# pymc-devs/nuts-rs

Measured on AMD Instinct MI355X. Metric: leapfrog-steps*dims/sec at 4096 chains x dim 1024 (post-warm-up NUTS draws), higher is better.
Workload: dtype f64; 1 GPU; K2: iid N(3,1) dim 1024 x 4096 chains per GPU, maxdepth 10, per-chain diag mass matrix, DiagNutsSettings defaults, num_tune 400 (untimed), seed 20260928; chains_per_gpu=4096, dim=1024, num_tune=400, parallelism=chains sharded x1, no collective, rng=ChaCha8 stream + ziggurat normals (reference semantics), draws_recorded=True, recorded_buffers_verified=True

## Files before the change

nuts_rs_amd/csrc/dev_math.hpp:

```cpp
#pragma once
#include <hip/hip_runtime.h>
#include <stdint.h>
#include "nuts_contract.hpp"
#include "detmath_tables.hpp"

namespace nm {

#define NM_DEV __device__ __forceinline__

#define NM_HD __host__ __device__ __forceinline__
NM_HD uint64_t d2u(double x) { return __builtin_bit_cast(uint64_t, x); }
NM_HD double u2d(uint64_t u) { return __builtin_bit_cast(double, u); }
#ifndef NM_TILE_MODE
#define NM_TILE_MODE 0
#endif
#define NM_ONE_WAVE_BLOCK (NM_TILE_MODE || blockDim.x == 64)
NM_DEV int lane_id() { return (int)(threadIdx.x & 63); }
NM_DEV void block_sync(bool single_wave) {
    if (single_wave || NM_TILE_MODE) asm volatile("" ::: "memory");
    else __syncthreads();
}
NM_DEV void chain_sync() { block_sync(false); }
NM_DEV int tid() { return NM_TILE_MODE ? (int)(threadIdx.x & 63) : (int)threadIdx.x; }
NM_DEV int wave_id() { return __builtin_amdgcn_readfirstlane((int)(threadIdx.x >> 6)); }
// ... 712 lines not shown
NM_DEV double fmin_rs(double a, double b) { return __builtin_fmin(a, b); }

NM_DEV void chacha8_block(const uint32_t* key, uint64_t counter, uint64_t stream, uint32_t (&out)[16]) {
    uint32_t s[16] = {0x61707865u, 0x3320646eu, 0x79622d32u, 0x6b206574u,
                      key[0], key[1], key[2], key[3], key[4], key[5], key[6], key[7],
                      (uint32_t)counter, (uint32_t)(counter >> 32), (uint32_t)stream, (uint32_t)(stream >> 32)};
    uint32_t x[16];
#pragma unroll
    for (int i = 0; i < 16; ++i) x[i] = s[i];
#define NM_QR(a, b, c, d)                                                   \
    x[a] += x[b]; x[d] ^= x[a]; x[d] = __builtin_rotateleft32(x[d], 16);    \
    x[c] += x[d]; x[b] ^= x[c]; x[b] = __builtin_rotateleft32(x[b], 12);    \
    x[a] += x[b]; x[d] ^= x[a]; x[d] = __builtin_rotateleft32(x[d], 8);     \
    x[c] += x[d]; x[b] ^= x[c]; x[b] = __builtin_rotateleft32(x[b], 7);
#pragma unroll
    for (int r = 0; r < 4; ++r) {
        NM_QR(0, 4, 8, 12) NM_QR(1, 5, 9, 13) NM_QR(2, 6, 10, 14) NM_QR(3, 7, 11, 15)
        NM_QR(0, 5, 10, 15) NM_QR(1, 6, 11, 12) NM_QR(2, 7, 8, 13) NM_QR(3, 4, 9, 14)
    }
#undef NM_QR
#pragma unroll
    for (int i = 0; i < 16; ++i) out[i] = x[i] + s[i];
}

constexpr int RNG_CACHE_WORDS = 512;
struct DevRng {
    const uint32_t* key;
    uint64_t pos;
    uint64_t base;
    uint32_t* cache;
    uint32_t cap;
    bool one_wave;

    NM_DEV void init(const uint32_t* k, uint64_t p, uint32_t* lds) {
        one_wave = NM_ONE_WAVE_BLOCK;
        key = k;
        pos = p;
        base = p + 16;
        cache = lds;
        cap = RNG_CACHE_WORDS;
    }
    NM_DEV bool has(uint64_t nwords) const { return pos >= base && (pos - base) + nwords <= (uint64_t)cap; }
    NM_DEV void refill() {
        block_sync(one_wave);
        base = pos & ~15ull;
        cap = RNG_CACHE_WORDS;
        if (tid() < RNG_CACHE_WORDS / 16) {
            uint32_t out[16];
            chacha8_block(key, (base >> 4) + (uint64_t)tid(), 0ull, out);
            uint4* dst = reinterpret_cast<uint4*>(cache + tid() * 16);
            dst[0] = make_uint4(out[0], out[1], out[2], out[3]);
            dst[1] = make_uint4(out[4], out[5], out[6], out[7]);
            dst[2] = make_uint4(out[8], out[9], out[10], out[11]);
            dst[3] = make_uint4(out[12], out[13], out[14], out[15]);
        }
        block_sync(one_wave);
    }
    NM_DEV uint32_t next_u32() {
        if (!has(1)) refill();
        uint32_t w = cache[pos - base];
        pos += 1;
        return w;
    }
    NM_DEV uint64_t next_u64() {
        if (!has(2)) refill();
        uint64_t lo = cache[pos - base], hi = cache[pos - base + 1];
        pos += 2;
        return (hi << 32) | lo;
    }
    NM_DEV bool random_bool_std() { return (int32_t)next_u32() < 0; }
    NM_DEV double random_f64() { return (double)(next_u64() >> 11) * (1.0 / 9007199254740992.0); }
    NM_DEV int random_bool(double p) {
        if (!(p >= 0.0 && p < 1.0)) return p == 1.0 ? 1 : -1;
        uint64_t p_int = (uint64_t)(p * 18446744073709551616.0);
        return next_u64() < p_int ? 1 : 0;
    }
};

struct ZigTables { const double* x; const double* f; };
constexpr double ZIG_R = 3.654152885361008796;

NM_DEV double normal_slow_path(DevRng& rng, uint64_t bits, ZigTables T) {
    for (;;) {
        int i = (int)(bits & 0xff);
        double u = u2d((bits >> 12) | 0x4000000000000000ull) - 3.0;
        double x = u * T.x[i];
        if (__builtin_fabs(x) < T.x[i + 1]) return x;
        if (i == 0) {
            double xx = 1.0, yy = 0.0;
            while (-2.0 * yy < xx * xx) {
                double a = u2d((rng.next_u64() >> 12) | 0x3ff0000000000000ull) - (1.0 - 2.220446049250313e-16 / 2.0);
                double b = u2d((rng.next_u64() >> 12) | 0x3ff0000000000000ull) - (1.0 - 2.220446049250313e-16 / 2.0);
                xx = ulog(a) / ZIG_R;
                yy = ulog(b);
            }
            return u < 0.0 ? xx - ZIG_R : ZIG_R - xx;
        }
        if (T.f[i + 1] + (T.f[i] - T.f[i + 1]) * rng.random_f64() < uexp(-x * x / 2.0)) return x;
        bits = rng.next_u64();
    }
}

NM_DEV void fill_standard_normals(DevRng& rng, double* stage, int count, ZigTables T) {
    const int lane = lane_id();
    int i = 0;
    while (i < count) {
        if (!rng.has(128)) rng.refill();
        const int nvalid = (count - i) < 64 ? (count - i) : 64;
        const uint32_t off = (uint32_t)(rng.pos - rng.base) + 2u * (uint32_t)lane;
        uint64_t bits = ((uint64_t)rng.cache[off + 1] << 32) | rng.cache[off];
        int zi = (int)(bits & 0xff);
        double u = u2d((bits >> 12) | 0x4000000000000000ull) - 3.0;
        double x = u * T.x[zi];
        bool ok = __builtin_fabs(x) < T.x[zi + 1];
        uint64_t fail = __ballot(lane < nvalid && !ok);
        int nacc = fail ? (int)__builtin_ctzll(fail) : nvalid;
        if (lane < nacc) stage[i + lane] = x;
        rng.pos += 2ull * (uint64_t)nacc;
        i += nacc;
        if (fail) {
            uint64_t fbits = wave_bcast_u64(bits, nacc);
            rng.pos += 2;
            double xs = normal_slow_path(rng, fbits, T);
            if (lane == 0) stage[i] = xs;
            i += 1;
        }
    }
    chain_sync();
}

constexpr int ZIG_FMAX = 64;
NM_DEV int uniform_i32(int x) { return __builtin_amdgcn_readfirstlane(x); }
NM_DEV int lane_get(int v, int idx) { return __builtin_amdgcn_readlane(v, idx); }
NM_DEV double lane_get_f64(double v, int idx) {
    const uint64_t b = d2u(v);
    const uint32_t lo = (uint32_t)__builtin_amdgcn_readlane((int)(uint32_t)b, idx);
    const uint32_t hi = (uint32_t)__builtin_amdgcn_readlane((int)(uint32_t)(b >> 32), idx);
    return u2d(((uint64_t)hi << 32) | lo);
}

#ifndef NM_PROF
#define NM_PROF 0
#endif
#if NM_PROF
#define NM_MARK_F(slot)                                                           \
    {                                                                             \
        const unsigned long long now_ = __builtin_amdgcn_s_memtime();             \
        if (blockIdx.x == 0 && threadIdx.x == 0) (void)__hip_atomic_fetch_add(&prof[slot], now_ - prof_t, __ATOMIC_RELAXED, __HIP_MEMORY_SCOPE_AGENT);     \
        prof_t = now_;                                                            \
    }
#else
#define NM_MARK_F(slot)
#endif
template <int P>
NM_DEV void fill_standard_normals_bulk(DevRng& rng, uint32_t* wbuf, double* samp, int count, ZigTables T, int nthreads,
                                       unsigned long long* prof, unsigned long long& prof_t) {
    static_assert(P <= 64, "rejection masks are kept one per lane");
    const int lane = lane_id();
    uint32_t* const small_cache = rng.cache;
    int produced = 0;
    block_sync(nthreads == 64);
    while (produced < count) {
        const int need = count - produced;
        int nc = need + ((need >> 4) > 8 ? (need >> 4) : 8);
        if (nc > 64 * P) nc = 64 * P;
        const uint64_t pos0 = rng.pos;
        const uint64_t b0 = pos0 >> 4;
        const int nb = (int)(((pos0 + 2ull * (uint64_t)nc - 1ull) >> 4) - b0) + 1;
        uint64_t* const lmask = reinterpret_cast<uint64_t*>(small_cache + 256);
        if (lane < 2 * P) lmask[lane] = 0ull;
        for (int b = tid(); b < nb; b += nthreads) {
            uint32_t out[16];
            chacha8_block(rng.key, b0 + (uint64_t)b, 0ull, out);
            uint4* dst = reinterpret_cast<uint4*>(wbuf + b * 16);
            dst[0] = make_uint4(out[0], out[1], out[2], out[3]);
            dst[1] = make_uint4(out[4], out[5], out[6], out[7]);
            dst[2] = make_uint4(out[8], out[9], out[10], out[11]);
            dst[3] = make_uint4(out[12], out[13], out[14], out[15]);
        }
        block_sync(nthreads == 64);
        NM_MARK_F(8)
        rng.cache = wbuf; rng.base = b0 << 4; rng.cap = (uint32_t)nb * 16u;
        const int w0 = (int)(pos0 - rng.base);
        double xr[P];
        int* const flist = reinterpret_cast<int*>(small_cache);
        int nrej = 0;
        {
            uint64_t cb[P];
            double tx[P], tn[P];
#pragma unroll
            for (int p = 0; p < P; ++p) {
                const int c = 64 * p + lane;
                cb[p] = ((uint64_t)wbuf[w0 + 2 * c + 1] << 32) | wbuf[w0 + 2 * c];
            }
#pragma unroll
            for (int p = 0; p < P; ++p) {
                const int zi = (int)(cb[p] & 0xff);
                tx[p] = T.x[zi];
                tn[p] = T.x[zi + 1];
            }
#pragma unroll
            for (int p = 0; p < P; ++p) {
                const int c = 64 * p + lane;
                const double u = u2d((cb[p] >> 12) | 0x4000000000000000ull) - 3.0;
                const double x = u * tx[p];
                const bool rej = !(__builtin_fabs(x) < tn[p]) && c < nc;
                xr[p] = x;
                const uint64_t fail = __ballot(rej);
                const int rank = nrej + (int)__builtin_amdgcn_mbcnt_hi((uint32_t)(fail >> 32),
                                                                       __builtin_amdgcn_mbcnt_lo((uint32_t)fail, 0u));
                flist[(rej && rank < ZIG_FMAX) ? rank : ZIG_FMAX + lane] = c;
                nrej += (int)__builtin_popcountll(fail);
            }
        }
        const int nlist = nrej < ZIG_FMAX ? nrej : ZIG_FMAX;
        int fcell, sp_r;
        double sp_x;
        bool sp_scalar;
        fcell = 0; sp_r = 0; sp_x = 0.0; sp_scalar = false;
        if (nlist > 0) {
            fcell = lane < nlist ? flist[lane] : 0;
            const int wa = w0 + 2 * fcell;
            const uint64_t bits0 = ((uint64_t)wbuf[wa + 1] << 32) | wbuf[wa];
            const uint64_t bits1 = ((uint64_t)wbuf[wa + 3] << 32) | wbuf[wa + 2];
            const uint64_t bits2 = ((uint64_t)wbuf[wa + 5] << 32) | wbuf[wa + 4];
            const int i0 = (int)(bits0 & 0xff);
            const double u0 = u2d((bits0 >> 12) | 0x4000000000000000ull) - 3.0;
            const double x0 = u0 * T.x[i0];
            const double u01 = (double)(bits1 >> 11) * (1.0 / 9007199254740992.0);
            const bool wedge = T.f[i0 + 1] + (T.f[i0] - T.f[i0 + 1]) * u01 < dexp(-x0 * x0 / 2.0);
            const int i2 = (int)(bits2 & 0xff);
            const double u2 = u2d((bits2 >> 12) | 0x4000000000000000ull) - 3.0;
            const double x2 = u2 * T.x[i2];
            const bool ok2 = __builtin_fabs(x2) < T.x[i2 + 1];
            sp_r = wedge ? 1 : 2;
            sp_x = wedge ? x0 : x2;
            sp_scalar = i0 == 0 || fcell + 2 >= nc || (!wedge && !ok2);
        }
        NM_MARK_F(9)
        NM_MARK_F(12)
        int cur = 0, j = 0, nf = 0;
        uint64_t sw = 0, nk = 0;
        int flj = 0;
        double flx = 0.0;
        bool open = true;
        const uint64_t scalar_mask = __ballot(sp_scalar);
        const int rr = lane < nlist ? sp_r : 0;
        const uint64_t m1 = __ballot(rr == 1), m2 = __ballot(rr == 2);
        const int s_before = (int)__builtin_amdgcn_mbcnt_hi((uint32_t)(m1 >> 32), __builtin_amdgcn_mbcnt_lo((uint32_t)m1, 0u)) +
                             2 * (int)__builtin_amdgcn_mbcnt_hi((uint32_t)(m2 >> 32), __builtin_amdgcn_mbcnt_lo((uint32_t)m2, 0u));
        const int prev_end = __builtin_amdgcn_update_dpp(-1, fcell + rr, 0x138, 0xf, 0xf, false);
        const bool chained = lane >= 1 && lane < nlist && fcell <= prev_end;
        const bool fast = scalar_mask == 0ull && nrej <= nlist && __ballot(chained) == 0ull;
        bool ev_active = false;
        int ev_j = 0;
        if (fast) {
            ev_j = fcell - s_before;
            ev_active = lane < nlist && ev_j < need;
            const uint64_t am = __ballot(ev_active);
            const int s_act = (int)__builtin_popcountll(m1 & am) + 2 * (int)__builtin_popcountll(m2 & am);
            j = (nc - s_act) < need ? (nc - s_act) : need;
            cur = j + s_act;
            if (ev_active) {
                const int q = fcell >> 6, off = fcell & 63;
                const uint64_t nk0 = ((1ull << (rr + 1)) - 1ull) << off;
                const uint64_t sw0 = off == 63 ? 0ull : (((1ull << rr) - 1ull) << (off + 1));
                (void)__hip_atomic_fetch_or(&lmask[q], sw0, __ATOMIC_RELAXED, __HIP_MEMORY_SCOPE_WORKGROUP);
                (void)__hip_atomic_fetch_or(&lmask[P + q], nk0, __ATOMIC_RELAXED, __HIP_MEMORY_SCOPE_WORKGROUP);
                const int spill = off + rr + 1 - 64;
                if (spill > 0) {
                    const uint64_t nx = (1ull << spill) - 1ull;
                    (void)__hip_atomic_fetch_or(&lmask[q + 1], nx, __ATOMIC_RELAXED, __HIP_MEMORY_SCOPE_WORKGROUP);
                    (void)__hip_atomic_fetch_or(&lmask[P + q + 1], nx, __ATOMIC_RELAXED, __HIP_MEMORY_SCOPE_WORKGROUP);
                }
            }
            sw = lane < P ? lmask[lane] : 0ull;
            nk = lane < P ? lmask[P + lane] : 0ull;
            open = false;
        }
        for (int g = 0; g < nlist && !fast; ++g) {
            const int f = lane_get(fcell, g);
            if (f < cur) continue;
            if (j + (f - cur) >= need) { cur += need - j; j = need; open = false; break; }
            j += f - cur;
            int r;
            double xs;
            if ((scalar_mask >> g) & 1ull) {
                const uint32_t lo = (uint32_t)uniform_i32((int)wbuf[w0 + 2 * f]);
                const uint32_t hi = (uint32_t)uniform_i32((int)wbuf[w0 + 2 * f + 1]);
                rng.pos = pos0 + 2ull * (uint64_t)(f + 1);
                xs = normal_slow_path(rng, ((uint64_t)hi << 32) | lo, T);
                r = (int)((rng.pos - pos0) >> 1) - (f + 1);
            } else {
                r = lane_get(sp_r, g);
                xs = lane_get_f64(sp_x, g);
            }
            for (int a = f, end = (f + 1 + r < 64 * P ? f + 1 + r : 64 * P); a < end;) {
                const int q = a >> 6, off = a & 63;
                const int take = (end - a) < (64 - off) ? (end - a) : (64 - off);
                const uint64_t bits = (take >= 64 ? ~0ull : ((1ull << take) - 1ull)) << off;
                const uint64_t sbits = a == f ? (bits & ~(1ull << off)) : bits;
                nk |= lane == q ? bits : 0ull;
                sw |= lane == q ? sbits : 0ull;
                a += take;
            }
            flj = lane == nf ? j : flj;
            flx = lane == nf ? xs : flx;
            nf += 1;
            j += 1;
            cur = f + 1 + r;
            if (j >= need || cur >= nc) { open = false; break; }
        }
        if (nrej > nlist && !fast) open = false;
        if (open && cur < nc) {
            const int take = (nc - cur) < (need - j) ? (nc - cur) : (need - j);
            j += take; cur += take;
        }
        rng.pos = pos0 + 2ull * (uint64_t)cur;
        NM_MARK_F(10)
        {
            double* const dummy = reinterpret_cast<double*>(small_cache) + 64 + lane;
            const int swlo = (int)(uint32_t)sw, swhi = (int)(uint32_t)(sw >> 32);
            const int nklo = (int)(uint32_t)nk, nkhi = (int)(uint32_t)(nk >> 32);
            int base = 0;
#pragma unroll
            for (int p = 0; p < P; ++p) {
                const uint32_t s_lo = (uint32_t)lane_get(swlo, p), s_hi = (uint32_t)lane_get(swhi, p);
                const uint64_t n_p = ((uint64_t)(uint32_t)lane_get(nkhi, p) << 32) | (uint32_t)lane_get(nklo, p);
                const int c = 64 * p + lane;
                const int below = (int)__builtin_amdgcn_mbcnt_hi(s_hi, __builtin_amdgcn_mbcnt_lo(s_lo, 0u));
                const bool keep = !((n_p >> lane) & 1ull) && c < cur;
                double* dst = keep ? samp + (produced + c - base - below) : dummy;
                *dst = xr[p];
                base += (int)__builtin_popcount(s_lo) + (int)__builtin_popcount(s_hi);
            }
            double* dst = fast ? (ev_active ? samp + (produced + ev_j) : dummy) : (lane < nf ? samp + (produced + flj) : dummy);
            *dst = fast ? sp_x : flx;
        }
        produced += j;
        block_sync(nthreads == 64);
// ... 24 lines not shown
```

nuts_rs_amd/csrc/nuts_kernels.hpp:

```cpp
#pragma once
#include <type_traits>
#include "nuts_contract.hpp"
#include "dev_math.hpp"
#include "../../include/nuts_amd.h"

namespace nm {

#ifndef NM_LDS_L1
#define NM_LDS_L1 1
#endif
constexpr int NM_CHECK_GROUP = 2;
#define NM_GROUP_BARRIER(m) do { if (((m) + 1) % NM_CHECK_GROUP == 0) __builtin_amdgcn_sched_barrier(0); } while (0)

constexpr bool plain_unit = !NM_TILE_MODE && !NM_CLUSTER_MODE;
template <int DPL, int W> constexpr bool reg_edges() { return plain_unit && W == 1 && (DPL == 16 || DPL == 2); }
template <int DPL, int W> constexpr bool batched_merges() { return batched_merges(DPL, W, plain_unit); }
template <int DPL, int W, class Dens> constexpr bool nog_mode();
constexpr int NM_TEST_CHUNK = 4;
constexpr int NM_TEST_CHUNK3_MAX = 2;

#ifndef NM_PROF
#define NM_PROF 0
#endif
#if NM_PROF
// ... 837 lines not shown
                o.v.a[k] = vh;
                o.z.a[k] = __builtin_fma(epsilon, vh, s.z.a[k]);
            }
            transform_to_x(C, o.z, x);
            o.logp = C.dens.template eval<DPL, W>(x, gx, C.dim, C.red);
            transform_to_gz(C, gx, o.g);
            double acc = 0.0;
#pragma unroll
            for (int k = 0; k < DPL; ++k) {
                o.v.a[k] = __builtin_fma(half, o.g.a[k], o.v.a[k]);
                acc = __builtin_fma(o.v.a[k], o.v.a[k], acc);
            }
            o.ke = 0.5 * C.red.sum(acc);
            if (x_out) *x_out = x;
            if (gx_out) *gx_out = gx;
            return;
        }
    }
    const double2* sg2 = C.tptr(C.lsig);
    const double2* mu2 = C.tptr(C.lmu);
    if constexpr (elementwise_trait<Dens>::value && plain_unit) {
        double acc = 0.0, kacc = 0.0;
        auto pass = [&](auto full_tile) __attribute__((always_inline)) {
            constexpr bool FULL = decltype(full_tile)::value;
            double2 sg = sg2[0], mm = mu2[0];
            [[maybe_unused]] double2 gg = make_double2(0., 0.);
            if constexpr (GMODE == 2) gg = C.ld2(gsrc.r, gsrc.so, 0);
#pragma unroll
            for (int m = 0; m < DPL / 2; ++m) {
                const double2 sg_c = sg, mm_c = mm;
                [[maybe_unused]] const double2 gg_c = gg;
                if (m + 1 < DPL / 2) { sg = sg2[(m + 1) * 64 * W]; mm = mu2[(m + 1) * 64 * W]; }
                if constexpr (GMODE == 2) { if (m + 1 < DPL / 2) gg = C.ld2(gsrc.r, gsrc.so, m + 1); }
#pragma unroll
                for (int j = 0; j < 2; ++j) {
                    const int k = 2 * m + j;
                    const double sgk = j ? sg_c.y : sg_c.x, muk = j ? mm_c.y : mm_c.x;
                    double gsk;
                    if constexpr (GMODE == 0) gsk = s.g.a[k];
                    else if constexpr (GMODE == 3) gsk = gshared->a[k];
                    else if constexpr (GMODE == 2) gsk = j ? gg_c.y : gg_c.x;
                    else {
                        const double ts = s.z.a[k] * sgk;
                        const double xs = __builtin_fma(1.0, muk, ts);
                        double unused_term;
                        const double gxs = C.dens.template elem<W, FULL>(xs, k, C.dim, unused_term);
                        gsk = gxs * sgk;
                    }
                    double vh, zk;
                    if constexpr (SITE == 2) {
                        asm("v_fma_f64 %0, %1, %2, %3" : "=v"(vh) : "v"(half), "v"(gsk), "v"(s.v.a[k]));
                        asm("v_fma_f64 %0, %1, %2, %3" : "=v"(zk) : "v"(epsilon), "v"(vh), "v"(s.z.a[k]));
                    } else {
                        vh = __builtin_fma(half, gsk, s.v.a[k]);
                        zk = __builtin_fma(epsilon, vh, s.z.a[k]);
                    }
                    o.z.a[k] = zk;
                    const double t = zk * sgk;
                    const double xk = __builtin_fma(1.0, muk, t);
                    double term;
                    const double gxk = C.dens.template elem<W, FULL>(xk, k, C.dim, term);
                    acc = acc + term;
                    const double gk = gxk * sgk;
                    if constexpr (GMODE == 0) o.g.a[k] = gk;
                    else gshared->a[k] = gk;
                    const double vk = __builtin_fma(half, gk, vh);
                    o.v.a[k] = vk;
                    kacc = __builtin_fma(vk, vk, kacc);
                    if (x_out) x_out->a[k] = xk;
                    if (gx_out) gx_out->a[k] = gxk;
                }
                __builtin_amdgcn_sched_barrier(0);
            }
        };
        if (C.dim == DPL * 64 * W) pass(std::true_type{}); else pass(std::false_type{});
        C.red.sum2(acc, kacc);
        o.logp = C.dens.finish(acc);
        o.ke = 0.5 * kacc;
        return;
    }
#pragma unroll
    for (int m = 0; m < DPL / 2; ++m) {
        const double2 sg = sg2[m * 64 * W], mm = mu2[m * 64 * W];
#pragma unroll
        for (int j = 0; j < 2; ++j) {
            const int k = 2 * m + j;
            double vh = __builtin_fma(half, s.g.a[k], s.v.a[k]);
            o.v.a[k] = vh;
            o.z.a[k] = __builtin_fma(epsilon, vh, s.z.a[k]);
            double t = o.z.a[k] * (j ? sg.y : sg.x);
            x.a[k] = __builtin_fma(1.0, (j ? mm.y : mm.x), t);
        }
    }
    o.logp = C.dens.template eval<DPL, W>(x, gx, C.dim, C.red);
    double acc = 0.0;
#pragma unroll
    for (int m = 0; m < DPL / 2; ++m) {
        const double2 sg = sg2[m * 64 * W];
#pragma unroll
        for (int j = 0; j < 2; ++j) {
            const int k = 2 * m + j;
            o.g.a[k] = gx.a[k] * (j ? sg.y : sg.x);
            o.v.a[k] = __builtin_fma(half, o.g.a[k], o.v.a[k]);
            acc = __builtin_fma(o.v.a[k], o.v.a[k], acc);
        }
    }
    o.ke = 0.5 * C.red.sum(acc);
    if (x_out) *x_out = x;
    if (gx_out) *gx_out = gx;
}

struct AcceptCollector {
    double initial_energy, sum, sum_sym, max_energy_error;
    uint64_t count;
    double pend_d;
    int npend;
    NM_DEV void register_init(double e0) {
        initial_energy = e0; sum = 0.; sum_sym = 0.; count = 0; max_energy_error = 0.;
        pend_d = 0.; npend = 0;
    }
    NM_DEV void flush() {
        if (npend == 0) return;
        const double d = lane_id() < npend ? pend_d : 0.0;
        const double e = dexp(fmin_rs(d, 0.));
        const double es = 2. * e / (1. + dexp(d));
        for (int i = 0; i < npend; ++i) {
            sum = sum + readlane_f64(e, i);
            sum_sym = sum_sym + readlane_f64(es, i);
        }
        npend = 0;
    }
    NM_DEV void register_divergent() {
        flush();
        sum = sum + 0.; sum_sym = sum_sym + 0.; count += 1; max_energy_error = -__builtin_inf();
    }
    NM_DEV void register_ok(double end_energy) {
        const double diff = initial_energy - end_energy;
        if (lane_id() == npend) pend_d = diff;
        npend += 1;
        count += 1;
        if (__builtin_fabs(diff) > __builtin_fabs(max_energy_error)) max_energy_error = diff;
        if (npend == 64) flush();
    }
    NM_DEV double mean() { flush(); return sum / (double)count; }
    NM_DEV double mean_sym() { flush(); return sum_sym / (double)count; }
};

NM_DEV void turn_acc(double zs, double vs, double ze, double ve, double& t1, double& t2) {
    double s = ze - zs;
    t1 = __builtin_fma(s, vs, t1);
    t2 = __builtin_fma(s, ve, t2);
}

template <int DPL, int W, class Dens>
NM_DEV void sample_velocity(ChainCtx<DPL, W, Dens>& C, Tile<DPL>& v, bool stage = true) {
#if NM_LDS_L1
#if NM_CLUSTER_MODE
    for (int j = 0; j < C.red.cl.k; ++j) {
        const int off = j * (int)C.P.cl_slice;
        const int cnt = C.gdim - off < (int)C.P.cl_slice ? C.gdim - off : (int)C.P.cl_slice;
        fill_standard_normals_bulk<(DPL * W + 1 < 17 ? DPL * W + 1 : 17)>(C.rng, reinterpret_cast<uint32_t*>(C.l1v), C.l1z, cnt, C.zig, 64 * W, C.P.prof, C.prof_t);
        if (j == C.red.cl.member) {
            const double2* s2 = C.tptr(C.l1z);
#pragma unroll
            for (int m = 0; m < DPL / 2; ++m) {
                const double2 q = s2[m * 64 * W];
                v.a[2 * m] = C.elem(2 * m) < C.dim ? 1.0 * q.x : 0.0;
                v.a[2 * m + 1] = C.elem(2 * m + 1) < C.dim ? 1.0 * q.y : 0.0;
            }
        }
        block_sync(false);
    }
    C.storeS(v, STAGE_V);
#else
    if (DPL == 2 && C.dim <= 48) {
        fill_standard_normals(C.rng, C.l1z, C.dim, C.zig);
    } else {
        fill_standard_normals_bulk<(DPL * W + 1 < 17 ? DPL * W + 1 : 17)>(C.rng, reinterpret_cast<uint32_t*>(C.l1v), C.l1z, C.dim, C.zig, 64 * W, C.P.prof, C.prof_t);
    }
    const double2* s2 = C.tptr(C.l1z);
#pragma unroll
    for (int m = 0; m < DPL / 2; ++m) {
        const double2 q = s2[m * 64 * W];
        v.a[2 * m] = C.elem(2 * m) < C.dim ? 1.0 * q.x : 0.0;
        v.a[2 * m + 1] = C.elem(2 * m + 1) < C.dim ? 1.0 * q.y : 0.0;
    }
    if (stage) C.storeS(v, STAGE_V);
#endif
#else
    fill_standard_normals(C.rng, C.sslot(STAGE_V), C.dim, C.zig);
    const int so = C.soS(STAGE_V);
#pragma unroll
    for (int m = 0; m < DPL / 2; ++m) {
        double2 q = C.ld2(C.rs, so, m);
        v.a[2 * m] = C.elem(2 * m) < C.dim ? 1.0 * q.x : 0.0;
        v.a[2 * m + 1] = C.elem(2 * m + 1) < C.dim ? 1.0 * q.y : 0.0;
    }
#endif
    block_sync(W == 1);
}

template <int DPL, int W>
NM_DEV double kinetic(const Tile<DPL>& v, Reducer<W>& R) {
    double acc = 0.0;
#pragma unroll
    for (int k = 0; k < DPL; ++k) acc = __builtin_fma(v.a[k], v.a[k], acc);
    return 0.5 * R.sum(acc);
}
template <int DPL, int W, class Dens>
NM_DEV double initial_kinetic(ChainCtx<DPL, W, Dens>& C, Tile<DPL>& v, bool stage = true) {
    if constexpr (kin_trait<Dens>::value) {
        if (C.sc.kin == NM_TRAJ_MICROCANONICAL) {
            normalize_tile(v, C.red);
            if (stage) C.storeS(v, STAGE_V);
            return 0.0;
        }
    }
    return kinetic(v, C.red);
}

template <int DPL, int W, class Dens>
NM_DEV double sum_ln_tile(ChainCtx<DPL, W, Dens>& C, const Tile<DPL>& t) {
    double acc = 0.0;
#pragma unroll
    for (int k = 0; k < DPL; ++k) {
        bool valid = C.elem(k) < C.dim;
        acc = acc + (valid ? dlog_impl<false>(valid ? t.a[k] : 1.0) : 0.0);
    }
    return C.red.sum(acc);
}


NM_DEV void stepsize_adapt_reset(ChainScalars& sc, const nm_settings& s, double initial_step) {
    sc.log_step = ulog(initial_step);
    if (s.step_size_method == NM_STEP_ADAM) {
        sc.adam_m = 0.; sc.adam_v = 0.; sc.adam_t = 0;
        return;
    }
    sc.log_step_adapted = sc.log_step;
    sc.hbar = 0.;
    sc.mu = ulog(10. * initial_step);
    sc.da_count = 1;
}

NM_DEV double powi_rs(double a, int32_t b) {
    uint32_t pw = b < 0 ? 0u - (uint32_t)b : (uint32_t)b;
    double mul = 1.0;
    for (;;) {
        if (pw & 1u) mul *= a;
        pw >>= 1;
        if (pw == 0) break;
        a *= a;
    }
    return b < 0 ? 1.0 / mul : mul;
}

}
#include "nuts_adapt.hpp"
namespace nm {

template <int DPL, int W, class Dens>
NM_DEV bool init_state(ChainCtx<DPL, W, Dens>& C, const Tile<DPL>& x, Pt<DPL>& st, Tile<DPL>& gx) {
    st.logp = C.dens.template eval<DPL, W>(x, gx, C.dim, C.red);
    if (dens_status(C) != 0) return false;
    if constexpr (lr_trait<Dens>::value) {
        transform_to_z(C, x, st.z);
        transform_to_gz(C, gx, st.g);
        bool ok_lr = true;
#pragma unroll
        for (int k = 0; k < DPL; ++k) {
            const bool valid = C.elem(k) < C.dim;
            ok_lr = ok_lr && (!valid || (is_finite(st.z.a[k]) && is_finite(st.g.a[k]) && st.g.a[k] != 0.0 &&
                                         is_finite(gx.a[k]) && is_finite(x.a[k])));
        }
        return C.red.all(ok_lr);
    }
    Tile<DPL> isig, sig, mu;
    C.loadP(isig, P_ISIG);
    C.load(sig, C.lsig);
    C.load(mu, C.lmu);
    bool ok = true;
#pragma unroll
    for (int k = 0; k < DPL; ++k) {
        double t = __builtin_fma(-1.0, mu.a[k], x.a[k]);
        st.z.a[k] = isig.a[k] * t;
        st.g.a[k] = gx.a[k] * sig.a[k];
        bool valid = C.elem(k) < C.dim;
        ok = ok && (!valid || (is_finite(st.z.a[k]) && is_finite(st.g.a[k]) && st.g.a[k] != 0.0 &&
                               is_finite(gx.a[k]) && is_finite(x.a[k])));
    }
    return C.red.all(ok);
}

template <int DPL, int W, class Dens>
NM_DEV uint64_t stepsize_init(ChainCtx<DPL, W, Dens>& C, const Tile<DPL>& x) {
    const nm_settings& s = C.P.s;
    if (s.step_size_method == NM_STEP_FIXED) { C.sc.step_size = s.fixed_step_size; return NM_CHAIN_OK; }
    Pt<DPL> st;
    {
        Tile<DPL> gx;
        if (!init_state(C, x, st, gx)) return dens_status(C) != 0 ? NM_CHAIN_LOGP_FATAL : NM_CHAIN_BAD_INIT;
    }
    const double logdet = C.sc.mm_logdet;
    sample_velocity(C, st.v);
    const double ke0 = initial_kinetic(C, st.v);
    st.ke = ke0;
    const double e0 = ke0 - (st.logp + logdet);
    AcceptCollector col;
    C.sc.step_size = s.initial_step;
    int dir = 0;
    for (int it = 0; it < 101; ++it) {
        Pt<DPL> o;
        const int sign = it == 0 ? 1 : dir;
        col.register_init(e0);
        leapfrog<DPL, W, Dens, 1>(C, st, o, (double)sign * C.sc.step_size * 1.0, (Tile<DPL>*)nullptr, (Tile<DPL>*)nullptr);
        const double energy = o.ke - (o.logp + logdet);
        const double err = energy - e0;
        if (dens_status(C) != 0) {
            if (it > 0) C.sc.step_size = s.initial_step;
            return NM_CHAIN_OK;
        }
        if (bad_energy(C, err, 1000.0)) {
            if (it > 0) C.sc.step_size = s.initial_step;
            return NM_CHAIN_OK;
        }
        col.register_ok(energy);
        const double accept = col.mean();
        if (it == 0) { dir = accept > s.target_accept ? 1 : -1; continue; }
        if (dir > 0) {
            if ((accept <= s.target_accept) | (C.sc.step_size > 1e5)) { stepsize_adapt_reset(C.sc, s, C.sc.step_size); return NM_CHAIN_OK; }
            C.sc.step_size *= 2.;
// ... 335 lines not shown
        }
        total = uniform_f64(mm.total);
        C.rng.pos += (uint64_t)(mmf & 2u);
        if (mmf & 4u) fatal = true;
        return (mmf & 1u) != 0;
    }
    const MergeOut mo = merge_math(a_log_size, b_log_size, is_main ? 1u : 0u, C.rng.cache[off_], C.rng.cache[off_ + 1]);
    total = uniform_f64(mo.total);
    const uint32_t mf = (uint32_t)__builtin_amdgcn_readfirstlane((int)mo.flags);
    C.rng.pos += (uint64_t)(mf & 2u);
    NM_MARK(C, 29)
    if (mf & 4u) fatal = true;
    return (mf & 1u) != 0;
}

struct DrawResult {
    uint64_t depth;
    bool diverging, reached_maxdepth, has_divergence_energy_error;
    bool has_div_end;
    double divergence_energy_error;
    int64_t div_start_idx;
    CandRef chosen;
    double e0;
};


NM_DEV bool turn_sign(bool fwd, double t) { return fwd ? t < 0. : t > 0.; }
NM_DEV bool turn_any6(bool fwd, double s1, double s2, double s3, double s4, double s5, double s6) {
    return fwd ? ((s1 < 0.) | (s2 < 0.) | (s3 < 0.) | (s4 < 0.) | (s5 < 0.) | (s6 < 0.))
               : ((s1 > 0.) | (s2 > 0.) | (s3 > 0.) | (s4 > 0.) | (s5 > 0.) | (s6 > 0.));
}
template <int DPL, int W>
NM_DEV bool turning_regs(const Pt<DPL>& a, const Pt<DPL>& b, bool fwd, Reducer<W>& R) {
    double s1 = 0., s2 = 0.;
#pragma unroll
    for (int k = 0; k < DPL; ++k) turn_acc(a.z.a[k], a.v.a[k], b.z.a[k], b.v.a[k], s1, s2);
    double s2v[2] = {s1, s2};
    return R.any_sign(s2v, fwd);
}

template <int DPL, int W, class Dens>
NM_DEV int cand_to_pool(ChainCtx<DPL, W, Dens>& C, uint32_t& used, const Tile<DPL>& z) {
    const int p = (int)__builtin_ctz(~used);
    used |= 1u << p;
    C.storeS_nt(z, slot_C(C.maxdepth_cfg, p));
    return p;
}

struct ChunkResult { double log_size; int cand_lane; bool fatal; };
NM_DEV double shfl_f64(double x, int src_lane) {
    const int lo = __shfl(__double2loint(x), src_lane), hi = __shfl(__double2hiint(x), src_lane);
    return __hiloint2double(hi, lo);
}
struct ChunkOut { double log_size; uint32_t packed; };
typedef const __attribute__((address_space(3))) uint32_t* lds_words_t;
NM_DEV ChunkOut resolve_chunk_core(double wv, uint32_t shape, lds_words_t words) {
    const int m = (int)(shape & 0xff), n_last = (int)((shape >> 8) & 0xff), k_last = (int)((shape >> 16) & 0xff);
    const int l = lane_id();
    const double ln2 = 0x1.62e42fefa39efp-1;
    double ls = wv;
    uint64_t pint[6];
    uint32_t need = 0, sure = 0, bad = 0, perf = 0;
#pragma unroll
    for (int k = 1; k <= 6; ++k) {
        pint[k - 1] = 0;
        if (k <= m) {
            const int h = 1 << (k - 1);
            const bool part = ((l + 1) & ((1 << k) - 1)) == 0;
            const bool done = part && (l < n_last || (l == n_last && k <= k_last));
            const double a = shfl_f64(ls, l - h), b = ls;
            const double diff = a - b;
            const double e = exp_sl(diff > 0. ? -diff : diff);
            const double lp = log1p_unit(e);
            const double total = a == b ? a + ln2 : (diff > 0. ? a + lp : (diff < 0. ? b + lp : diff));
            const bool ge = b >= total;
            const double p_ = exp_sl(b - total);
            const bool in01 = p_ >= 0.0 && p_ < 1.0;
            pint[k - 1] = in01 ? (uint64_t)(p_ * 18446744073709551616.0) : 0ull;
            if (done) {
                perf |= 1u << k;
                if (ge || (!in01 && p_ == 1.0)) sure |= 1u << k;
                else if (in01) need |= 1u << k;
                else bad |= 1u << k;
            }
            if (part) ls = total;
        }
    }
    const uint32_t fatal = __ballot(bad != 0) != 0ull ? 1u : 0u;
    uint32_t before = 0, total_words = 0;
#pragma unroll
    for (int k = 1; k <= 6; ++k) {
        const uint64_t bm = __ballot((need >> k) & 1u);
        before += __builtin_amdgcn_mbcnt_hi((uint32_t)(bm >> 32), __builtin_amdgcn_mbcnt_lo((uint32_t)bm, 0u));
        total_words += 2u * (uint32_t)__builtin_popcountll(bm);
    }
    uint32_t take = sure;
#pragma unroll
    for (int k = 1; k <= 6; ++k) {
        if ((need >> k) & 1u) {
            const uint32_t q = before + (uint32_t)__builtin_popcount(need & ((1u << k) - 1u));
            const uint64_t w = ((uint64_t)words[2u * q + 1u] << 32) | words[2u * q];
            if (w < pint[k - 1]) take |= 1u << k;
        }
    }
    int cand = l;
#pragma unroll
    for (int k = 1; k <= 6; ++k) {
        if (k <= m) {
            const int from = __shfl(cand, l - (1 << (k - 1)));
            if ((perf >> k) & 1u) cand = ((take >> k) & 1u) ? cand : from;
        }
    }
    const int top = (1 << m) - 1;
    ChunkOut R;
    R.log_size = readlane_f64(ls, top);
    R.packed = (uint32_t)__builtin_amdgcn_readlane(cand, top) | (fatal << 8) | ((uint32_t)__builtin_amdgcn_readfirstlane((int)total_words) << 16);
    return R;
}
template <int DPL, int W, class Dens>
NM_DEV ChunkResult resolve_chunk(ChainCtx<DPL, W, Dens>& C, double wv, int m, int n_last, int k_last) {
    if (!C.rng.has(128)) C.rng.refill();
    const ChunkOut o = resolve_chunk_core(wv, (uint32_t)m | ((uint32_t)n_last << 8) | ((uint32_t)k_last << 16),
                                          (lds_words_t)(C.rng.cache + (uint32_t)(C.rng.pos - C.rng.base)));
    C.rng.pos += (uint64_t)(o.packed >> 16);
    ChunkResult R;
    R.log_size = uniform_f64(o.log_size);
    R.cand_lane = __builtin_amdgcn_readfirstlane((int)(o.packed & 0xff));
    R.fatal = ((o.packed >> 8) & 1u) != 0;
    return R;
}
template <int DPL, int W, class Dens>
NM_DEV int ring_to_pool(ChainCtx<DPL, W, Dens>& C, uint32_t& used, int ring_lane) {
    Tile<DPL> z;
    C.loadS(z, slot_R(C.maxdepth_cfg, ring_lane));
    return cand_to_pool(C, used, z);
}

template <int DPL, int W, class Dens, bool SAMPLING = false>
NM_DEV uint64_t nuts_transition(ChainCtx<DPL, W, Dens>& C, AcceptCollector& col, DrawResult& R, Tile<DPL>& zc) {
    const nm_settings& s = C.P.s;
    ChainScalars& sc = C.sc;
    const int MD = C.maxdepth_cfg;
    Pt<DPL> E, O;
    constexpr bool RE = reg_edges<DPL, W>();
    constexpr bool NOG = nog_mode<DPL, W, Dens>();
    constexpr bool FD = false;
    constexpr int TCH = (DPL == 16 && W == 1) ? NM_TEST_CHUNK : 0;
    constexpr bool ROLL = SAMPLING && TCH > 0;
    [[maybe_unused]] Tile<DPL> Gsh;
    [[maybe_unused]] Tile<DPL>* const gsh = &Gsh;
    [[maybe_unused]] Tile<DPL> FDz, FDv;
    [[maybe_unused]] EdgeTile<DPL> MLz, MLv, MRz, MRv;
    NM_MARK(C, 0)
    sample_velocity(C, E.v, !RE);
    NM_MARK(C, 1)
    if (sc.mm_id != sc.transform_id) {
        Tile<DPL> x, gx, isig, sig, mu;
        C.loadP(x, P_X);
        C.loadP(gx, P_GX);
        if constexpr (lr_trait<Dens>::value) {
            transform_to_z(C, x, E.z);
            if constexpr (tile_trait<Dens>::value) C.dens.tile_skip_density();
            transform_to_gz(C, gx, E.g);
        } else {
        C.loadP(isig, P_ISIG);
        C.load(sig, C.lsig);
        C.load(mu, C.lmu);
#pragma unroll
        for (int k = 0; k < DPL; ++k) {
            double t = __builtin_fma(-1.0, mu.a[k], x.a[k]);
            E.z.a[k] = isig.a[k] * t;
            E.g.a[k] = gx.a[k] * sig.a[k];
        }
        }
        C.storeP(E.z, P_Z);
        C.storeP(E.g, P_GZ);
        sc.logdet = sc.mm_logdet;
        sc.transform_id = sc.mm_id;
    } else {
        C.loadP(E.z, P_Z);
        if constexpr (!NOG) C.loadP(E.g, P_GZ);
    }
    const double logdet = sc.logdet;
    const double ke_init = initial_kinetic(C, E.v, !RE);
    E.ke = ke_init;
    if constexpr (RE) { MLz.put(E.z); MLv.put(E.v); MRz.put(E.z); MRv.put(E.v); }
    const double e0 = ke_init - (sc.logp + logdet);
    R.e0 = e0;
    col.register_init(e0);
    int left_slot = 0, right_slot = 0;
    bool o_is_edge = false;
    int o_edge_sign = 0;
    uint64_t depth = 0;
    double log_size = 0.;
    int64_t left_idx = 0, right_idx = 0;
    [[maybe_unused]] double left_ke = ke_init, right_ke = ke_init;
    CandRef mc = {-1, sc.logp, ke_init, 0};
    uint32_t used = 0;
    constexpr bool BATCH = batched_merges<DPL, W>();
    [[maybe_unused]] double wv = 0., lpv = 0., kev = 0.;

    uint64_t mindepth = s.mindepth, maxdepth = s.maxdepth;
    if (s.has_target_integration_time) {
        double q = __builtin_ceil(s.target_integration_time / sc.step_size);
        uint64_t max_steps = q >= 18446744073709551616.0 ? ~0ull : (q > 0 ? (uint64_t)q : 0ull);
        uint64_t fl = 63 - __builtin_clzll(max_steps | 1ull);
        uint64_t ce = ((max_steps & (max_steps - 1)) == 0) ? fl : fl + 1;
        mindepth = fl > s.mindepth ? fl : s.mindepth;
        uint64_t xd = ce > mindepth ? ce : mindepth;
        maxdepth = xd < s.maxdepth ? xd : s.maxdepth;
    }
    const double max_energy_error = pin_scalar(s.max_energy_error);
    R.diverging = false; R.reached_maxdepth = false; R.has_divergence_energy_error = false; R.has_div_end = true;
    R.divergence_energy_error = 0.; R.div_start_idx = 0;
    const bool want_div = C.P.out_div_start || C.P.out_div_start_grad || C.P.out_div_end;
    bool fatal = false;
    bool in_extra = false;
    uint64_t extra_left = 0;
    int sign = 1;

    for (;;) {
        bool check;
        if (!in_extra) {
            if (C.P.dim == 0) break;
            if (!(depth < maxdepth)) { R.reached_maxdepth = true; break; }
            sign = C.rng.random_bool_std() ? 1 : -1;
            check = (s.check_turning != 0) && !(depth < mindepth);
        } else {
            if (extra_left == 0) break;
            extra_left -= 1;
            check = false;
        }
        NM_MARK(C, 24)
        const bool fwd = sign > 0;
        const int64_t edge_idx = fwd ? right_idx : left_idx;
        const uint64_t nleaf = 1ull << depth;
        const uint32_t used_before = used;
        const double epsilon = (double)sign * sc.step_size * 1.0;
        int stop = STOP_NONE;
        double sub_log_size = 0.;
        CandRef sub_cand = {-2, 0., 0., 0};
        const bool reuse_edge = o_is_edge && o_edge_sign == sign;
        o_is_edge = false;

#define NM_LEAF_ACCOUNT(START, PT, WOUT, LOGIDX)                                                          \
        {                                                                                                 \
            const double energy_ = (PT).ke - ((PT).logp + logdet);                                        \
            const double err_ = energy_ - e0;                                                             \
            const int dst_ = dens_status(C);             \
            if (dst_ == 2) { stop = STOP_FATAL; }                                                         \
            else if (dst_ == 1) {               \
                col.register_divergent();                                                                 \
                R.diverging = true; R.has_divergence_energy_error = false; R.has_div_end = false;         \
                R.div_start_idx = (PT).idx - (int64_t)sign;                                               \
                if (want_div) C.storeS((START).z, slot_F(0));                                             \
                stop = STOP_DIVERGING;                                                                    \
            } else                                                                                        \
            if (bad_energy(C, err_, max_energy_error)) {                                                  \
                col.register_divergent();                                                                 \
                R.diverging = true; R.has_divergence_energy_error = true; R.divergence_energy_error = err_; \
                R.div_start_idx = (PT).idx - (int64_t)sign;                                               \
                if (want_div) {           \
                    C.storeS((START).z, slot_F(0)); C.storeS((PT).z, slot_F(0) + 1);                      \
                }                                                                                         \
                stop = STOP_DIVERGING;                                                                    \
            } else {                                                                                      \
                col.register_ok(energy_);                                                                 \
                WOUT = -err_;                                                                             \
                if constexpr (SAMPLING) leaf_log_put(C, (uint32_t)(LOGIDX), WOUT);                        \
            }                                                                                             \
        }

        auto top_level_turning = [&]() __attribute__((always_inline)) -> bool {
                double s1 = 0., s2 = 0., s3 = 0., s4 = 0., s5 = 0., s6 = 0.;
                const auto mlz = C.edge_z(left_slot), mlv = C.edge_v(left_slot);
                const auto mrz = C.edge_z(right_slot), mrv = C.edge_v(right_slot);
                if (depth == 0) {
                    return turning_regs(E, O, fwd, C.red);
                } else {
                    const int so_ofz = C.soS(slot_F((int)depth)), so_ofv = C.soS(slot_F((int)depth) + 1);
                    const bool of_in_regs = depth == 1;
                    auto rows = [&](auto far_is_left, auto of_regs) __attribute__((always_inline)) {
                        constexpr bool OFR = decltype(of_regs)::value;
                        auto row = [&](int m, double2 oz, double2 ov) __attribute__((always_inline)) {
                            double2 lz, lv, rz, rv;
                            if constexpr (RE) {
                                lz = MLz.pair(m); lv = MLv.pair(m); rz = MRz.pair(m); rv = MRv.pair(m);
                            } else {
                                lz = C.ld2(mlz.r, mlz.so, m); lv = C.ld2(mlv.r, mlv.so, m);
                                rz = C.ld2(mrz.r, mrz.so, m); rv = C.ld2(mrv.r, mrv.so, m);
                            }
                            const double cz0 = O.z.a[2 * m], cz1 = O.z.a[2 * m + 1];
                            const double cv0 = O.v.a[2 * m], cv1 = O.v.a[2 * m + 1];
                            turn_acc(lz.x, lv.x, cz0, cv0, s1, s2); turn_acc(lz.y, lv.y, cz1, cv1, s1, s2);
                            turn_acc(rz.x, rv.x, cz0, cv0, s3, s4); turn_acc(rz.y, rv.y, cz1, cv1, s3, s4);
                            if constexpr (decltype(far_is_left)::value) { turn_acc(lz.x, lv.x, oz.x, ov.x, s5, s6); turn_acc(lz.y, lv.y, oz.y, ov.y, s5, s6); }
                            else { turn_acc(rz.x, rv.x, oz.x, ov.x, s5, s6); turn_acc(rz.y, rv.y, oz.y, ov.y, s5, s6); }
                        };
                        if constexpr (!OFR && ROLL) {
                            double2 ozb[TCH > 0 ? TCH : 1], ovb[TCH > 0 ? TCH : 1];
#pragma unroll
                            for (int c = 0; c < TCH; ++c) { ozb[c] = C.ld2(C.rs, so_ofz, c); ovb[c] = C.ld2(C.rs, so_ofv, c); }
                            __builtin_amdgcn_sched_barrier(0);
#pragma unroll
                            for (int m = 0; m < DPL / 2; ++m) {
                                row(m, ozb[m % TCH], ovb[m % TCH]);
                                if (m + TCH < DPL / 2) { ozb[m % TCH] = C.ld2(C.rs, so_ofz, m + TCH); ovb[m % TCH] = C.ld2(C.rs, so_ofv, m + TCH); }
// ... 1150 lines not shown
```

Baseline: 280.0 billion leapfrog-steps*dims/s.

## Interleave ChaCha block generation with ziggurat table lookups in sampling velocity draw

Adds a pipelined variant of the bulk normal generator, used only in the sampling phase with single-wave chains. Each lane computes one ChaCha block per pass, and later passes are interleaved with ziggurat table-lookup groups of up to eight cells, separated by scheduling barriers. This is meant to hide the latency of the table loads behind ChaCha arithmetic and to avoid the single strided block loop. The cost is a fixed three-pass schedule, more register pressure, and reliance on one wave covering all the blocks. Correctness depends on later groups only reading words from passes already written.

```diff
diff --git a/nuts_rs_amd/csrc/dev_math.hpp b/nuts_rs_amd/csrc/dev_math.hpp
--- a/nuts_rs_amd/csrc/dev_math.hpp
+++ b/nuts_rs_amd/csrc/dev_math.hpp
@@ -888,10 +888,44 @@
 #else
 #define NM_MARK_F(slot)
 #endif
-template <int P>
+constexpr int ZIG_GROUP = 8;
+template <int P0, int P1>
+NM_DEV void zig_request(const uint32_t* wbuf, int w0, int lane, ZigTables T, uint64_t (&cb)[ZIG_GROUP], double (&tx)[ZIG_GROUP], double (&tn)[ZIG_GROUP]) {
+    static_assert(P1 - P0 <= ZIG_GROUP, "one landing register set per cell pass of the group");
+#pragma unroll
+    for (int p = P0; p < P1; ++p) {
+        const int c = 64 * p + lane;
+        cb[p - P0] = ((uint64_t)wbuf[w0 + 2 * c + 1] << 32) | wbuf[w0 + 2 * c];
+    }
+#pragma unroll
+    for (int p = P0; p < P1; ++p) {
+        const int zi = (int)(cb[p - P0] & 0xff);
+        tx[p - P0] = T.x[zi];
+        tn[p - P0] = T.x[zi + 1];
+    }
+}
+template <int P0, int P1, int P>
+NM_DEV void zig_finish(const uint64_t (&cb)[ZIG_GROUP], const double (&tx)[ZIG_GROUP], const double (&tn)[ZIG_GROUP], int lane, int nc, int* flist,
+                       double (&xr)[P], int& nrej) {
+#pragma unroll
+    for (int p = P0; p < P1; ++p) {
+        const int c = 64 * p + lane;
+        const double u = u2d((cb[p - P0] >> 12) | 0x4000000000000000ull) - 3.0;
+        const double x = u * tx[p - P0];
+        const bool rej = !(__builtin_fabs(x) < tn[p - P0]) && c < nc;
+        xr[p] = x;
+        const uint64_t fail = __ballot(rej);
+        const int rank = nrej + (int)__builtin_amdgcn_mbcnt_hi((uint32_t)(fail >> 32), __builtin_amdgcn_mbcnt_lo((uint32_t)fail, 0u));
+        flist[(rej && rank < ZIG_FMAX) ? rank : ZIG_FMAX + lane] = c;
+        nrej += (int)__builtin_popcountll(fail);
+    }
+}
+
+template <int P, bool PIPE = false>
 NM_DEV void fill_standard_normals_bulk(DevRng& rng, uint32_t* wbuf, double* samp, int count, ZigTables T, int nthreads,
                                        unsigned long long* prof, unsigned long long& prof_t) {
     static_assert(P <= 64, "rejection masks are kept one per lane");
+    static_assert(!PIPE || P <= 23, "the pipelined chunk has three ChaCha passes: 3072 words");
     const int lane = lane_id();
     uint32_t* const small_cache = rng.cache;
     int produced = 0;
@@ -905,6 +939,19 @@
         const int nb = (int)(((pos0 + 2ull * (uint64_t)nc - 1ull) >> 4) - b0) + 1;
         uint64_t* const lmask = reinterpret_cast<uint64_t*>(small_cache + 256);
         if (lane < 2 * P) lmask[lane] = 0ull;
+        [[maybe_unused]] auto chacha_pass = [&](int b) __attribute__((always_inline)) {
+            if (b < nb) {
+                uint32_t out[16];
+                chacha8_block(rng.key, b0 + (uint64_t)b, 0ull, out);
+                uint4* dst = reinterpret_cast<uint4*>(wbuf + b * 16);
+                dst[0] = make_uint4(out[0], out[1], out[2], out[3]);
+                dst[1] = make_uint4(out[4], out[5], out[6], out[7]);
+                dst[2] = make_uint4(out[8], out[9], out[10], out[11]);
+                dst[3] = make_uint4(out[12], out[13], out[14], out[15]);
+            }
+        };
+        if constexpr (PIPE) chacha_pass(lane);
+        else
         for (int b = tid(); b < nb; b += nthreads) {
             uint32_t out[16];
             chacha8_block(rng.key, b0 + (uint64_t)b, 0ull, out);
@@ -921,7 +968,29 @@
         double xr[P];
         int* const flist = reinterpret_cast<int*>(small_cache);
         int nrej = 0;
-        {
+        if constexpr (PIPE) {
+            constexpr int G0 = P < 7 ? P : 7, G1 = P < 15 ? P : 15;
+            uint64_t cb[ZIG_GROUP];
+            double tx[ZIG_GROUP], tn[ZIG_GROUP];
+            zig_request<0, G0>(wbuf, w0, lane, T, cb, tx, tn);
+            __builtin_amdgcn_sched_barrier(0);
+            chacha_pass(64 + lane);
+            __builtin_amdgcn_sched_barrier(0);
+            zig_finish<0, G0, P>(cb, tx, tn, lane, nc, flist, xr, nrej);
+            if constexpr (G0 < P) {
+                zig_request<G0, G1>(wbuf, w0, lane, T, cb, tx, tn);
+                __builtin_amdgcn_sched_barrier(0);
+                if constexpr (128 * P + 15 > 2048) {
+                    chacha_pass(128 + lane);
+                    __builtin_amdgcn_sched_barrier(0);
+                }
+                zig_finish<G0, G1, P>(cb, tx, tn, lane, nc, flist, xr, nrej);
+            }
+            if constexpr (G1 < P) {
+                zig_request<G1, P>(wbuf, w0, lane, T, cb, tx, tn);
+                zig_finish<G1, P, P>(cb, tx, tn, lane, nc, flist, xr, nrej);
+            }
+        } else {
             uint64_t cb[P];
             double tx[P], tn[P];
 #pragma unroll
diff --git a/nuts_rs_amd/csrc/nuts_kernels.hpp b/nuts_rs_amd/csrc/nuts_kernels.hpp
--- a/nuts_rs_amd/csrc/nuts_kernels.hpp
+++ b/nuts_rs_amd/csrc/nuts_kernels.hpp
@@ -1013,7 +1013,7 @@
     t2 = __builtin_fma(s, ve, t2);
 }
 
-template <int DPL, int W, class Dens>
+template <int DPL, int W, class Dens, bool PIPE = false>
 NM_DEV void sample_velocity(ChainCtx<DPL, W, Dens>& C, Tile<DPL>& v, bool stage = true) {
 #if NM_LDS_L1
 #if NM_CLUSTER_MODE
@@ -1037,7 +1037,7 @@
     if (DPL == 2 && C.dim <= 48) {
         fill_standard_normals(C.rng, C.l1z, C.dim, C.zig);
     } else {
-        fill_standard_normals_bulk<(DPL * W + 1 < 17 ? DPL * W + 1 : 17)>(C.rng, reinterpret_cast<uint32_t*>(C.l1v), C.l1z, C.dim, C.zig, 64 * W, C.P.prof, C.prof_t);
+        fill_standard_normals_bulk<(DPL * W + 1 < 17 ? DPL * W + 1 : 17), PIPE>(C.rng, reinterpret_cast<uint32_t*>(C.l1v), C.l1z, C.dim, C.zig, 64 * W, C.P.prof, C.prof_t);
     }
     const double2* s2 = C.tptr(C.l1z);
 #pragma unroll
@@ -1679,7 +1679,7 @@
     [[maybe_unused]] Tile<DPL> FDz, FDv;
     [[maybe_unused]] EdgeTile<DPL> MLz, MLv, MRz, MRv;
     NM_MARK(C, 0)
-    sample_velocity(C, E.v, !RE);
+    sample_velocity<DPL, W, Dens, SAMPLING && W == 1>(C, E.v, !RE);
     NM_MARK(C, 1)
     if (sc.mm_id != sc.transform_id) {
         Tile<DPL> x, gx, isig, sig, mu;
```

New measurement: 277.1 billion leapfrog-steps*dims/s. -1.0%, worse.
